# google/telluride_decoding

Hardware: AMD Instinct MI355X
Metric: TRF-fit samples/sec (higher is better)
Workload: dtype f32 (every product as 3 float16 products of a 2-piece split on the f16 MFMA, f32 accumulate, f64 slab sums; f64 solve)

## Files before the change

telluride_decoding_amd/csrc/lagcov.hip:

```cpp
#include <cstdlib>
#include <cstring>

#include "td_common.h"

namespace {

typedef float f32x16 __attribute__((ext_vector_type(16)));

constexpr int kThreads = 256;
constexpr int kTile = 128;
constexpr int kTileG = 64;
constexpr int kNpfU = 10;
constexpr int kNpfU2 = 13;
constexpr int kNpfG = 9;
constexpr int kLagsPerWg = 8;
constexpr int kHalo = 8;
constexpr size_t kLagcovScratchCap = size_t(256) << 20;

__device__ __forceinline__ int xcd_remap(int bid, int nwg) {
  const int q = nwg >> 3, r = nwg & 7;
  const int xcd = bid & 7, within = bid >> 3;
  const int base = xcd < r ? xcd * (q + 1) : r * (q + 1) + (xcd - r) * q;
  return base + within;
}
// ... 140 lines not shown
    }
  };
  const int nfull = nk >> 1;
  float c[6], n[6];
  ld(0, c);
  int kk = 0;
  for (; kk + 1 < nfull; kk += 2) {
    ld(kk + 1, n);
    mm(c);
    ld(kk + 2 < nfull ? kk + 2 : kk + 1, c);
    mm(n);
  }
  if (kk < nfull) mm(c);
  if (nk & 1) {
    ld(nfull, c);
    if (lk) { c[0] = 0.f; c[1] = 0.f; }
    mm(c);
  }
}

template <int kTileT, bool kM2, bool kN2>
__device__ __forceinline__ void mfma_tile_few(const float* __restrict__ as,
                                              const float* __restrict__ bs, int wave, int lane,
                                              int nk, int g, int lg, f32x16 (&acc)[2][2][2]) {
  const int lr = lane & 31, lk = lane >> 5;
  const int s_phases = 8 >> lg;
  const int nfull = nk >> 1;
#pragma unroll
  for (int le = 0; le < 2; ++le) {
    const int slot = 2 * wave + le;
    const int lag = slot & (g - 1), phase = slot >> lg;
    const float* ap = as + lk * 64 + lr;
    const float* bp = bs + (lk + lag) * 64 + lr;
    auto step = [&](int kk, bool tail) {
      const bool live = !tail || lk == 0;
      const float a0 = live ? ap[kk * 128] : 0.f;
      const float a1 = (kM2 && live) ? ap[kk * 128 + 32] : 0.f;
      const float b0 = bp[kk * 128];
      acc[le][0][0] = __builtin_amdgcn_mfma_f32_32x32x2f32(a0, b0, acc[le][0][0], 0, 0, 0);
      if (kM2) acc[le][1][0] = __builtin_amdgcn_mfma_f32_32x32x2f32(a1, b0, acc[le][1][0], 0, 0, 0);
      if (kN2) {
        const float b1 = bp[kk * 128 + 32];
        acc[le][0][1] = __builtin_amdgcn_mfma_f32_32x32x2f32(a0, b1, acc[le][0][1], 0, 0, 0);
        if (kM2) acc[le][1][1] = __builtin_amdgcn_mfma_f32_32x32x2f32(a1, b1, acc[le][1][1], 0, 0, 0);
      }
    };
#pragma unroll 4
    for (int kk = phase; kk < nfull; kk += s_phases) step(kk, false);
    if ((nk & 1) && (nfull & (s_phases - 1)) == phase) step(nfull, true);
  }
}

template <bool kUnified, int kTileT, int kNPF, bool kVec4, bool kFew>
__global__ __launch_bounds__(kThreads, 2) void lagcov_mfma_kernel(LagParams p) {
  extern __shared__ __attribute__((aligned(16))) float lds[];

  const int tid = threadIdx.x;
  const int lane = tid & 63;
  const int wave = __builtin_amdgcn_readfirstlane(tid >> 6);

  int id = xcd_remap(blockIdx.x, gridDim.x);
  const int group = id % p.n_groups; id /= p.n_groups;
  const int cbt = id % p.n_cbt; id /= p.n_cbt;
  const int cat = id % p.n_cat; id /= p.n_cat;
  const LagWork w = p.works[id];
  const int e0 = p.e_min + group * (kFew ? p.lag_g : kLagsPerWg);

  const int rows = kUnified ? kTileT + kHalo + e0 : 2 * kTileT + kHalo;
  const float* as = lds;
  const float* bs = kUnified ? lds + e0 * 64 : lds + kTileT * 64;

  const int ca_eff = p.ca + p.a_ones;
  const bool m2 = ca_eff - cat * 64 > 32;
  const bool n2 = p.cb - cbt * 64 > 32;
  const int ones_col = p.a_ones ? p.ca - cat * 64 : -1;

  f32x16 acc[2][2][2];
#pragma unroll
  for (int i = 0; i < 2; ++i)
#pragma unroll
    for (int j = 0; j < 2; ++j)
#pragma unroll
      for (int k = 0; k < 2; ++k)
#pragma unroll
        for (int r = 0; r < 16; ++r) acc[i][j][k][r] = 0.f;

  float4 pf[kNPF];
  prefetch_tile<kUnified, kTileT, kNPF, kVec4>(p, w, w.u_begin, e0, rows, cat, cbt, tid, pf);
  store_tile<kUnified, kTileT, kNPF>(lds, w, w.u_begin, ones_col, tid, pf);
  __syncthreads();

  for (long long ut = w.u_begin; ut < w.u_end; ut += kTileT) {
    const bool more = ut + kTileT < w.u_end;
    if (more)
      prefetch_tile<kUnified, kTileT, kNPF, kVec4>(p, w, ut + kTileT, e0, rows, cat, cbt, tid,
                                                      pf);
    const long long left = w.u_end - ut;
    const int nk = (kUnified && left < kTileT) ? (int)left : kTileT;
    if (kFew) {
      if (m2) {
        if (n2) mfma_tile_few<kTileT, true, true>(as, bs, wave, lane, nk, p.lag_g, p.lag_lg, acc);
        else    mfma_tile_few<kTileT, true, false>(as, bs, wave, lane, nk, p.lag_g, p.lag_lg, acc);
      } else {
        if (n2) mfma_tile_few<kTileT, false, true>(as, bs, wave, lane, nk, p.lag_g, p.lag_lg, acc);
        else    mfma_tile_few<kTileT, false, false>(as, bs, wave, lane, nk, p.lag_g, p.lag_lg, acc);
      }
    } else if (m2) {
      if (n2) mfma_tile<kTileT, true, true>(as, bs, wave, lane, nk, acc);
      else    mfma_tile<kTileT, true, false>(as, bs, wave, lane, nk, acc);
    } else {
      if (n2) mfma_tile<kTileT, false, true>(as, bs, wave, lane, nk, acc);
      else    mfma_tile<kTileT, false, false>(as, bs, wave, lane, nk, acc);
    }
    if (more) {
      __syncthreads();
      store_tile<kUnified, kTileT, kNPF>(lds, w, ut + kTileT, ones_col, tid, pf);
      __syncthreads();
    }
  }

  const int lr = lane & 31, lk = lane >> 5;
  float* slab = p.partial + (size_t)id * p.e_pad * p.ca_pad * p.cb_pad;
#pragma unroll
  for (int le = 0; le < 2; ++le) {
    int e_idx = group * kLagsPerWg + 2 * wave + le;
    if (kFew) {
      const int slot = 2 * wave + le;
      e_idx = ((slot >> p.lag_lg) * p.n_groups + group) * p.lag_g + (slot & (p.lag_g - 1));
    }
    float* pe = slab + (size_t)e_idx * p.ca_pad * p.cb_pad;
#pragma unroll
    for (int m = 0; m < 2; ++m)
#pragma unroll
      for (int n = 0; n < 2; ++n)
#pragma unroll
        for (int r = 0; r < 16; ++r) {
          const int i = cat * 64 + m * 32 + (r & 3) + 8 * (r >> 2) + 4 * lk;
          const int j = cbt * 64 + n * 32 + lr;
          pe[(size_t)i * p.cb_pad + j] = acc[le][m][n][r];
        }
  }
}

constexpr int kBfTile = 128;
template <int kRowDw, int kPieces> struct BfGeom {
  static constexpr int kRows = kRowDw == 83 ? 160 : 192;
  static constexpr int kPieceDw = 64 * kRowDw;
  static constexpr size_t kLdsBytes =
      sizeof(unsigned) * (2 * kPieces * kPieceDw + (kPieces == 2 ? 2 * 2 * 96 + 8 * 1024 : 0));
};
constexpr int kBfThreads = 512;

typedef td_u32x4 u32x4;

__device__ __forceinline__ float comp4(const float4& v, int q) {
  return q == 0 ? v.x : q == 1 ? v.y : q == 2 ? v.z : v.w;
}

template <bool kZero, int kBfPieceDw, bool kF16>
__device__ __forceinline__ void bf_kstep(const unsigned* __restrict__ ap,
                                         const unsigned* __restrict__ bp,
                                         const unsigned* a_mask, f32x16 (&acc)[4]) {
  constexpr int kP = kF16 ? 2 : 3;
  u32x4 a[kP];
  unsigned d[kP][6];
#pragma unroll
  for (int pc = 0; pc < kP; ++pc) {
#pragma unroll
    for (int i = 0; i < 4; ++i) a[pc][i] = ap[pc * kBfPieceDw + i];
#pragma unroll
    for (int i = 0; i < 6; ++i) d[pc][i] = bp[pc * kBfPieceDw + i];
  }
  if (a_mask) {
#pragma unroll
    for (int pc = 0; pc < kP; ++pc)
#pragma unroll
      for (int i = 0; i < 4; ++i) a[pc][i] &= a_mask[i];
  }
  u32x4 b[4][kP];
#pragma unroll
  for (int pc = 0; pc < kP; ++pc)
#pragma unroll
    for (int i = 0; i < 4; ++i) {
      b[0][pc][i] = d[pc][i];
      b[1][pc][i] = __builtin_amdgcn_alignbit(d[pc][i + 1], d[pc][i], 16);
      b[2][pc][i] = d[pc][i + 1];
      b[3][pc][i] = __builtin_amdgcn_alignbit(d[pc][i + 2], d[pc][i + 1], 16);
    }
  f32x16 c[4];
#pragma unroll
  for (int r = 0; r < 4; ++r) {
    if (kZero) {
#pragma unroll
      for (int k = 0; k < 16; ++k) c[r][k] = 0.f;
    } else {
      c[r] = acc[r];
    }
  }
  if constexpr (kF16) {
    constexpr int pa[3] = {1, 0, 0}, pb[3] = {0, 1, 0};
#pragma unroll
    for (int t = 0; t < 3; ++t)
#pragma unroll
      for (int r = 0; r < 4; ++r) c[r] = td_mfma_f16(a[pa[t] % kP], b[r][pb[t] % kP], c[r]);
  } else {
    constexpr int pa[6] = {2, 0, 1, 1, 0, 0}, pb[6] = {0, 2, 1, 0, 1, 0};
#pragma unroll
    for (int t = 0; t < 6; ++t)
#pragma unroll
      for (int r = 0; r < 4; ++r) c[r] = td_mfma_bf16(a[pa[t] % kP], b[r][pb[t] % kP], c[r]);
  }
#pragma unroll
  for (int r = 0; r < 4; ++r) acc[r] = c[r];
}

template <int kFrom, int kTo, int kBfPieceDw, bool kF16, int kChain>
__device__ __forceinline__ void bf_ksteps(const unsigned* __restrict__ ap,
                                          const unsigned* __restrict__ bp, f32x16 (&acc)[4],
                                          f32x16 (&total)[4]) {
#pragma unroll
  for (int s = kFrom; s < kTo; ++s) {
    if (s % kChain == 0) bf_kstep<true, kBfPieceDw, kF16>(ap + 8 * s, bp + 8 * s, nullptr, acc);
    else                 bf_kstep<false, kBfPieceDw, kF16>(ap + 8 * s, bp + 8 * s, nullptr, acc);
    if ((s + 1) % kChain == 0) {
#pragma unroll
      for (int r = 0; r < 4; ++r) total[r] += acc[r];
    }
    __builtin_amdgcn_sched_barrier(0);
  }
}

template <bool kVec4, int kBfRowDw, bool kF16, bool kVirt = false, bool kKs = false>
__global__ __launch_bounds__(kBfThreads) void lagcov_split_kernel(LagParams p) {
  static_assert(!kVirt || kF16, "virtual images: the float16 form");
  static_assert(!kKs || kVirt, "shared tasks: virtual images");
  constexpr int kChain = 8;
  constexpr int kP = kF16 ? 2 : 3;
  extern __shared__ __attribute__((aligned(16))) unsigned ldsu[];
  constexpr int kBfRows = BfGeom<kBfRowDw, kP>::kRows;
  constexpr int kBfPieceDw = BfGeom<kBfRowDw, kP>::kPieceDw;

  const int tid = threadIdx.x;
  const int lane = tid & 63;
  const int wave = __builtin_amdgcn_readfirstlane(tid >> 6);
  int quad = wave & 1, mt = (wave >> 1) & 1, nt = wave >> 2;

  int id = xcd_remap(blockIdx.x, gridDim.x);
  const int group = id % p.n_groups; id /= p.n_groups;
  const int part = id;
  LagWork w = p.works[id];
  const int e0 = group * kLagsPerWg;
  int lag_off = e0 + 4 * quad, out_lag = lag_off;
  bool active = true, a_ext = false;
  const VirtImage* img = nullptr;
  VirtSeg vs = {0, 0, 0};
  int kparts = 1, kq = 0;
  if constexpr (kVirt) {
    const VirtGroup* vg = p.vgroups + group;
    const VirtTask tk = vg->task[wave];
    img = p.vimgs + vg->image;
    mt = tk.mt; nt = tk.nt; lag_off = tk.lag0; out_lag = tk.out_lag;
    active = out_lag >= 0; a_ext = tk.a_ext != 0;
    if constexpr (kKs) {
      kparts = __builtin_amdgcn_readfirstlane((int)tk.kparts);
      kq = __builtin_amdgcn_readfirstlane((int)tk.kq);
    }
    vs = p.vsegs[id];
  }
  const int ksn = 8 / kparts, ks0 = kq * ksn;

  f32x16 total[4];
#pragma unroll
  for (int r = 0; r < 4; ++r)
#pragma unroll
    for (int k = 0; k < 16; ++k) total[r][k] = 0.f;

  const int c4 = (tid & 15) * 4, rg = tid >> 4;
  const bool has_tail = kBfRows == 192 || wave < 4;
  const bool early = wave < 4;
  float sc[4] = {1.f, 1.f, 1.f, 1.f};
  int vdesc[4] = {0, 0, 0, 0};
  if constexpr (kVirt) {
#pragma unroll
    for (int q = 0; q < 4; ++q) {
      const int k = kVec4 ? c4 + q : lane;
      vdesc[q] = (img->src[k] + 1) | (img->role[k] ? 0x100 : 0) | ((int)img->shift[k] << 16);
    }
  }
  constexpr int kVPairs = kBfRows / 16;
  auto v_src = [&](int q) { return (vdesc[q] & 0xff) - 1; };
  auto v_sh = [&](int q) { return vdesc[q] >> 16; };
  auto v_role = [&](int q) { return (vdesc[q] & 0x100) != 0; };
  if (kF16) {
#pragma unroll
    for (int q = 0; q < 4; ++q) {
      const int ch = kVirt ? v_src(q) : min(c4 + q, 63);
      const int k = ch >= 0 ? td_f16_scale_exp(td_chan_max_of(p.chan_max, ch)) : 0;
      sc[q] = __builtin_bit_cast(float, (unsigned)(127 + k) << 23);
      if (kVirt && ch < 0) sc[q] = 0.f;
    }
    if (blockIdx.x == 0 && tid < 128) {
      unsigned* all = const_cast<unsigned*>(p.chan_max);
      const unsigned m = td_chan_max_of(p.chan_max, tid);
      all[kChanShards * 128 + tid] = m;
      if (p.scale_out) p.scale_out[tid] = m;
    }
    if (p.zero_tab && blockIdx.x == (gridDim.x > 1 ? 1 : 0))
      for (int i = tid; i < kChanTab; i += kBfThreads) p.zero_tab[i] = 0u;
  }
  const bool never = false;
  float anchor_a = 0.f, anchor_b = 1.f;
  auto sched_anchor = [&](unsigned* dst) {
    if (!never || tid >= 160) return;
    reinterpret_cast<unsigned short*>(dst)[tid] = (unsigned short)(anchor_a * anchor_b);
  };
  float4 pf[6];
  auto interior = [&](long long ut) -> bool {
    return kVec4 && p.ca == 64 && ut >= 0 && ut + kBfRows <= w.a_valid;
  };
  auto vrange = [&](long long ut, int q, int& lo, int& hi) {
    const long long lim = 1 << 20;
    const long long a0 = -ut, b0 = w.a_valid - ut;
    const long long a1 = vs.seg_begin - ut, b1 = (vs.seg_end < w.a_valid ? vs.seg_end : w.a_valid) - ut;
    const int a0i = (int)(a0 < -lim ? -lim : (a0 > lim ? lim : a0)), b0i = (int)(b0 < -lim ? -lim : (b0 > lim ? lim : b0));
    const int a1i = (int)(a1 < -lim ? -lim : (a1 > lim ? lim : a1)), b1i = (int)(b1 < -lim ? -lim : (b1 > lim ? lim : b1));
    lo = (v_role(q) ? a1i : a0i) - v_sh(q);
    hi = (v_role(q) ? b1i : b0i) - v_sh(q);
    if (v_src(q) < 0) { lo = 0; hi = 0; }
  };
  int v_min_shift = 0, v_max_shift = 0;
  bool v_any_role1 = false;
  if constexpr (kVirt) { v_min_shift = img->min_shift; v_max_shift = img->max_shift; v_any_role1 = img->any_role1 != 0; }
  auto vinside = [&](long long ut) -> bool {
    const long long lo = v_any_role1 && vs.seg_begin > 0 ? vs.seg_begin : 0;
    const long long hi = v_any_role1 && vs.seg_end < w.a_valid ? vs.seg_end : w.a_valid;
    return ut + v_min_shift >= lo && ut + kBfRows + v_max_shift <= hi;
  };
  auto prefetch_to = [&](long long ut, float4 (&pfr)[6]) {
    if constexpr (kVirt) {
      if (vinside(ut)) {
        const int ld = (int)p.lda;
        const float* base = p.a + (w.a_row0 + ut) * p.lda;
        if (kVec4) {
          const int off = (4 * rg + v_sh(0)) * ld + (v_src(0) < 0 ? 0 : v_src(0));
#pragma unroll
          for (int s = 0; s < 4; ++s) pfr[s] = *reinterpret_cast<const float4*>(base + s * ld + off);
          if (has_tail) {
            const float* tb = base + kBfTile * ld;
            const int toff = off - 2 * rg * ld;
#pragma unroll
            for (int s = 0; s < 2; ++s) pfr[4 + s] = *reinterpret_cast<const float4*>(tb + s * ld + toff);
          }
        } else {
          const int off = (2 * wave + v_sh(0)) * ld + (v_src(0) < 0 ? 0 : v_src(0));
          float* pv = reinterpret_cast<float*>(&pfr[0]);
#pragma unroll
          for (int j = 0; j < kVPairs; ++j) {
            pv[2 * j] = (base + 16 * j * ld)[off];
            pv[2 * j + 1] = (base + (16 * j + 1) * ld)[off];
          }
        }
        return;
      }
      const float* base = p.a + (w.a_row0 + ut) * p.lda;
      const int ld = (int)p.lda;
      const long long l0 = -ut, h0 = w.a_valid - 1 - ut, lim = 1 << 20;
      const int rlo = (int)(l0 < -lim ? -lim : (l0 > lim ? lim : l0));
      const int rhi = (int)(h0 < -lim ? -lim : (h0 > lim ? lim : h0));
      if (kVec4) {
        const int src = v_src(0) < 0 ? 0 : v_src(0), sh = v_sh(0);
#pragma unroll
        for (int s = 0; s < 4; ++s) {
          const int rc = max(rlo, min(4 * rg + s + sh, rhi));
          pfr[s] = *reinterpret_cast<const float4*>(base + rc * ld + src);
        }
        if (has_tail) {
#pragma unroll
          for (int s = 0; s < 2; ++s) {
            const int rc = max(rlo, min(kBfTile + 2 * rg + s + sh, rhi));
            pfr[4 + s] = *reinterpret_cast<const float4*>(base + rc * ld + src);
          }
        }
      } else {
        const int src = v_src(0) < 0 ? 0 : v_src(0), sh = v_sh(0);
        float* pv = reinterpret_cast<float*>(&pfr[0]);
#pragma unroll
        for (int j = 0; j < 2 * kVPairs; ++j) {
          const int r = 16 * (j >> 1) + 2 * wave + (j & 1);
          const int rc = max(rlo, min(r + sh, rhi));
          pv[j] = base[rc * ld + src];
        }
      }
      return;
    }
    if (interior(ut)) {
      const float* base = p.a + (w.a_row0 + ut) * p.lda + c4;
      const int ld = (int)p.lda;
#pragma unroll
      for (int s = 0; s < 4; ++s)
        pfr[s] = *reinterpret_cast<const float4*>(base + (4 * rg + s) * ld);
      if (has_tail) {
#pragma unroll
        for (int s = 0; s < 2; ++s)
          pfr[4 + s] = *reinterpret_cast<const float4*>(base + (kBfTile + 2 * rg + s) * ld);
      }
      return;
    }
    const RowWindow rw = row_window(p.a, p.lda, w.a_row0, ut, w.a_valid, 0, p.ca);
#pragma unroll
    for (int s = 0; s < 4; ++s) pfr[s] = load_row4_raw<kVec4>(rw, 4 * rg + s, c4);
    if (has_tail) {
#pragma unroll
      for (int s = 0; s < 2; ++s) pfr[4 + s] = load_row4_raw<kVec4>(rw, kBfTile + 2 * rg + s, c4);
    }
  };
  auto prefetch = [&](long long ut) { prefetch_to(ut, pf); };
  auto store_from = [&](long long ut, unsigned* buf, const float4 (&pfr)[6]) {
    if constexpr (kVirt && !kVec4) {
      const float* pv = reinterpret_cast<const float*>(&pfr[0]);
      unsigned* dst = buf + lane * kBfRowDw + wave;
      if (vinside(ut)) {
#pragma unroll
        for (int j = 0; j < kVPairs; ++j) {
          unsigned h, l;
          td_split2_f16(pv[2 * j] * sc[0], pv[2 * j + 1] * sc[0], h, l);
          dst[8 * j] = h;
          dst[kBfPieceDw + 8 * j] = l;
        }
        return;
      }
      int lo, hi;
      vrange(ut, 0, lo, hi);
#pragma unroll
      for (int j = 0; j < kVPairs; ++j) {
        const int r = 16 * j + 2 * wave;
        const float x0 = (r >= lo && r < hi) ? pv[2 * j] : 0.f;
        const float x1 = (r + 1 >= lo && r + 1 < hi) ? pv[2 * j + 1] : 0.f;
        unsigned h, l;
        td_split2_f16(x0 * sc[0], x1 * sc[0], h, l);
        dst[8 * j] = h;
        dst[kBfPieceDw + 8 * j] = l;
      }
      return;
    }
    float4 v[6];
#pragma unroll
    for (int s = 0; s < 6; ++s) v[s] = pfr[s];
    if constexpr (kVirt) {
      if (!vinside(ut))
#pragma unroll
      for (int q = 0; q < 4; ++q) {
        int lo, hi;
        vrange(ut, kVec4 ? 0 : q, lo, hi);
        if (lo <= 0 && hi >= kBfRows) continue;
#pragma unroll
        for (int s = 0; s < 4; ++s) {
          const int r = 4 * rg + s;
          float& x = reinterpret_cast<float*>(&v[s])[q];
          x = (r >= lo && r < hi) ? x : 0.f;
        }
#pragma unroll
        for (int s = 0; s < 2; ++s) {
          const int r = kBfTile + 2 * rg + s;
          float& x = reinterpret_cast<float*>(&v[4 + s])[q];
          x = (r >= lo && r < hi) ? x : 0.f;
        }
      }
    } else
    if (!interior(ut)) {
      const RowWindow rw = row_window(p.a, p.lda, w.a_row0, ut, w.a_valid, 0, p.ca);
#pragma unroll
      for (int s = 0; s < 4; ++s) v[s] = mask_row4(rw, 4 * rg + s, true, c4, pfr[s]);
      if (has_tail) {
#pragma unroll
        for (int s = 0; s < 2; ++s) v[4 + s] = mask_row4(rw, kBfTile + 2 * rg + s, true, c4, pfr[4 + s]);
      }
    }
#pragma unroll
    for (int q = 0; q < 4; ++q) {
      unsigned* dst = buf + (c4 + q) * kBfRowDw + 2 * rg;
      if (kF16) {
        unsigned h[2], l[2];
#pragma unroll
        for (int d = 0; d < 2; ++d)
          td_split2_f16(comp4(v[2 * d], q) * sc[q], comp4(v[2 * d + 1], q) * sc[q], h[d], l[d]);
        dst[0] = h[0]; dst[1] = h[1];
        dst[kBfPieceDw] = l[0]; dst[kBfPieceDw + 1] = l[1];
      } else {
        unsigned h[2], m[2], l[2];
#pragma unroll
        for (int d = 0; d < 2; ++d)
          td_split3(comp4(v[2 * d], q), comp4(v[2 * d + 1], q), h[d], m[d], l[d]);
        dst[0] = h[0]; dst[1] = h[1];
        dst[kBfPieceDw] = m[0]; dst[kBfPieceDw + 1] = m[1];
        dst[(kP - 1) * kBfPieceDw] = l[0]; dst[(kP - 1) * kBfPieceDw + 1] = l[1];
      }
    }
    if (has_tail) {
#pragma unroll
      for (int q = 0; q < 4; ++q) {
        unsigned* tail = buf + (c4 + q) * kBfRowDw + kBfTile / 2 + rg;
        if (kF16) {
          unsigned h, l;
          td_split2_f16(comp4(v[4], q) * sc[q], comp4(v[5], q) * sc[q], h, l);
          tail[0] = h;
          tail[kBfPieceDw] = l;
        } else {
          unsigned h, m, l;
          td_split3(comp4(v[4], q), comp4(v[5], q), h, m, l);
          tail[0] = h;
          tail[kBfPieceDw] = m;
          tail[(kP - 1) * kBfPieceDw] = l;
        }
      }
    }
  };
  auto store = [&](long long ut, unsigned* buf) { store_from(ut, buf, pf); };

  const int lj = lane & 31, lg = lane >> 5;
  const int a_off = (mt * 32 + lj) * kBfRowDw + 4 * lg;
  const int b_off = (nt * 32 + lj) * kBfRowDw + 4 * lg + (lag_off >> 1);

  f32x16 acc[4];
  unsigned* const buf0 = ldsu;
  unsigned* const buf1 = ldsu + kP * kBfPieceDw;
  for (; id < p.n_work; id += p.n_part) {
  if (id != part) {
    __syncthreads();
    w = p.works[id];
    if constexpr (kVirt) vs = p.vsegs[id];
  }
  if constexpr (kKs) {
    const long long u_stop = vs.u_end_ext;
    float4 pf2[6];
    prefetch_to(w.u_begin, pf);
    store_from(w.u_begin, buf0, pf);
    if (w.u_begin + kBfTile < u_stop) prefetch_to(w.u_begin + kBfTile, pf);
    __syncthreads();
    auto ks_tile = [&](long long ut, const unsigned* cur, unsigned* nxt, float4 (&pfa)[6], float4 (&pfb)[6]) {
      const bool more = ut + kBfTile < u_stop;
      if (ut + 2 * kBfTile < u_stop) prefetch_to(ut + 2 * kBfTile, pfb);
      long long left = (a_ext ? u_stop : w.u_end) - ut;
      if (!active) left = 0;
      const unsigned* ap = cur + a_off;
      const unsigned* bp = cur + b_off;
      if (left >= kBfTile) {
        bf_kstep<true, kBfPieceDw, kF16>(ap + 8 * ks0, bp + 8 * ks0, nullptr, acc);
        for (int s = ks0 + 1; s < ks0 + ksn; ++s)
          bf_kstep<false, kBfPieceDw, kF16>(ap + 8 * s, bp + 8 * s, nullptr, acc);
#pragma unroll
        for (int r = 0; r < 4; ++r) total[r] += acc[r];
      } else if (left > 16 * ks0) {
        const int nk = (int)left;
#pragma unroll
        for (int r = 0; r < 4; ++r)
#pragma unroll
          for (int k = 0; k < 16; ++k) acc[r][k] = 0.f;
        const int t_hi = min(nk, 16 * (ks0 + ksn));
        for (int t0 = 16 * ks0; t0 < t_hi; t0 += 16) {
          const int cnt = nk - t0 - 8 * lg;
          unsigned mask[4];
#pragma unroll
          for (int d = 0; d < 4; ++d)
            mask[d] = cnt >= 2 * d + 2 ? 0xffffffffu : cnt == 2 * d + 1 ? 0x0000ffffu : 0u;
          bf_kstep<false, kBfPieceDw, kF16>(ap + (t0 >> 1), bp + (t0 >> 1), mask, acc);
        }
#pragma unroll
        for (int r = 0; r < 4; ++r) total[r] += acc[r];
      }
      if (more) {
        store_from(ut + kBfTile, nxt, pfa);
        __syncthreads();
      }
    };
    for (long long ut = w.u_begin; ut < u_stop; ut += 2 * kBfTile) {
      ks_tile(ut, buf0, buf1, pf, pf2);
      if (ut + kBfTile < u_stop) ks_tile(ut + kBfTile, buf1, buf0, pf2, pf);
    }
    continue;
  }
  prefetch(w.u_begin);
  store(w.u_begin, buf0);
  __syncthreads();

  const long long u_stop = kVirt ? vs.u_end_ext : w.u_end;
  int parity = 0;
  for (long long ut = w.u_begin; ut < u_stop; ut += kBfTile, parity ^= 1) {
    const unsigned* cur = parity ? buf1 : buf0;
    unsigned* nxt = parity ? buf0 : buf1;
    const bool more = ut + kBfTile < u_stop;
    if (more) prefetch(ut + kBfTile);
    long long left = w.u_end - ut;
    if constexpr (kVirt) {
      if (a_ext) left = u_stop - ut;
      if (!active) left = 0;
      if (left < kBfTile && more) store(ut + kBfTile, nxt);
    }
    const unsigned* ap = cur + a_off;
    const unsigned* bp = cur + b_off;
    if (left >= kBfTile) {
      bf_ksteps<0, 2, kBfPieceDw, kF16, kChain>(ap, bp, acc, total);
      if (more && early) { store(ut + kBfTile, nxt); sched_anchor(nxt); }
      bf_ksteps<2, 6, kBfPieceDw, kF16, kChain>(ap, bp, acc, total);
      if (more && !early) { store(ut + kBfTile, nxt); sched_anchor(nxt); }
      bf_ksteps<6, 8, kBfPieceDw, kF16, kChain>(ap, bp, acc, total);
    } else {
      const int nk = (int)left;
#pragma unroll
      for (int r = 0; r < 4; ++r)
#pragma unroll
        for (int k = 0; k < 16; ++k) acc[r][k] = 0.f;
      for (int t0 = 0; t0 < nk; t0 += 16) {
        const int cnt = nk - t0 - 8 * lg;
        unsigned mask[4];
#pragma unroll
        for (int d = 0; d < 4; ++d)
          mask[d] = cnt >= 2 * d + 2 ? 0xffffffffu : cnt == 2 * d + 1 ? 0x0000ffffu : 0u;
        bf_kstep<false, kBfPieceDw, kF16>(ap + (t0 >> 1), bp + (t0 >> 1), mask, acc);
      }
#pragma unroll
      for (int r = 0; r < 4; ++r) total[r] += acc[r];
    }
    if (more) __syncthreads();
  }
  }

  if constexpr (kKs) {
    float* const red = reinterpret_cast<float*>(ldsu);
    const int task = wave / kparts;
    for (int step = kparts >> 1; step >= 1; step >>= 1) {
      __syncthreads();
      if (kq >= step && kq < 2 * step) {
        float* dst = red + (size_t)(task * step + kq - step) * 4096 + lane;
#pragma unroll
        for (int r = 0; r < 4; ++r)
#pragma unroll
          for (int k = 0; k < 16; ++k) dst[(r * 16 + k) * 64] = total[r][k];
      }
      __syncthreads();
      if (kq < step) {
        const float* src = red + (size_t)(task * step + kq) * 4096 + lane;
#pragma unroll
        for (int r = 0; r < 4; ++r)
#pragma unroll
          for (int k = 0; k < 16; ++k) total[r][k] += src[(r * 16 + k) * 64];
      }
    }
    active = active && kq == 0;
  }
  if constexpr (kVirt) {
    if (active) {
      float* slab = p.partial + (size_t)part * p.slab_elems;
      const int lr = lane & 31, lk = lane >> 5;
#pragma unroll
      for (int r = 0; r < 4; ++r) {
        float* pe = slab + (size_t)(out_lag + r) * 1024;
#pragma unroll
        for (int k = 0; k < 16; ++k) pe[((k & 3) + 8 * (k >> 2) + 4 * lk) * 32 + lr] = total[r][k];
      }
    }
    return;
  }
  float* slab = p.partial + (size_t)part * p.e_pad * p.ca_pad * p.cb_pad;
#pragma unroll
  for (int r = 0; r < 4; ++r) {
    float* pe = slab + (size_t)(e0 + 4 * quad + r) * p.ca_pad * p.cb_pad;
    const int lr = lane & 31, lk = lane >> 5;
#pragma unroll
    for (int k = 0; k < 16; ++k) {
      const int i = mt * 32 + (k & 3) + 8 * (k >> 2) + 4 * lk;
      const int j = nt * 32 + lr;
      pe[(size_t)i * p.cb_pad + j] = total[r][k];
    }
  }
}

struct Narrow16Params {
  const float* x;
  const float* y;
  long long ldx, ldy;
  int c, d, pre, l1;
  const LagWork* works;
  int n_lg, lpw;
  int do_main, do_tgt;
  float* part;
  float* tpart;
  double* csum;
  double* ysum;
  long long n_part;
};

typedef float n16_f32x4 __attribute__((ext_vector_type(4)));

__device__ __forceinline__ float n16_load(__amdgpu_buffer_rsrc_t rs, unsigned voff) {
  return __builtin_bit_cast(float, __builtin_amdgcn_raw_buffer_load_b32(rs, (int)voff, 0, 0));
}

template <bool kMain, bool kTgt, int kLpw, int kD, bool kPre>
__global__ __launch_bounds__(256) void lagcov_narrow16_kernel(Narrow16Params p) {
  const int tid = threadIdx.x, lane = tid & 63;
  const int wave = __builtin_amdgcn_readfirstlane(tid >> 6);
  const int g = wave % p.n_lg, sub = wave / p.n_lg, n_sub = 4 / p.n_lg;
  const LagWork w = p.works[blockIdx.x];
  const long long len = w.u_end - w.u_begin;
  const long long sub_len = ((len + n_sub - 1) / n_sub + 3) / 4 * 4;
  const long long ub = w.u_begin + sub * sub_len;
  const long long ue = ub + sub_len < w.u_end ? ub + sub_len : w.u_end;
  const int j = lane & 15, k = lane >> 4;
  const int e0 = g * kLpw;
  const int ne = p.l1 - e0 < kLpw ? p.l1 - e0 : kLpw;
  const __amdgpu_buffer_rsrc_t rx = __builtin_amdgcn_make_buffer_rsrc(
      const_cast<float*>(p.x + w.b_row0 * p.ldx), 0,
      w.b_valid > 0 ? (int)(((w.b_valid - 1) * p.ldx + p.c) * 4) : 0, 0x00020000);
  const __amdgpu_buffer_rsrc_t ry = __builtin_amdgcn_make_buffer_rsrc(
      const_cast<float*>(p.y + w.a_row0 * p.ldy), 0,
      w.a_valid > 0 ? (int)(((w.a_valid - 1) * p.ldy + p.d) * 4) : 0, 0x00020000);
  const unsigned row_x = (unsigned)(p.ldx * 4), row_y = (unsigned)(p.ldy * 4);
  const unsigned lane_x = j < p.c ? (unsigned)k * row_x + 4u * j : 0x80000000u;
  const unsigned lane_y = (unsigned)k * row_y;
  const unsigned lag0 = (unsigned)e0 * row_x, pre_x = (unsigned)p.pre * row_x;
  n16_f32x4 acc[kLpw];
  float tacc[kD][kLpw];
#pragma unroll
  for (int q = 0; q < kLpw; ++q) {
    acc[q] = n16_f32x4{0.f, 0.f, 0.f, 0.f};
#pragma unroll
    for (int col = 0; col < kD; ++col) tacc[col][q] = 0.f;
  }
  float cs = 0.f, ys[kD];
#pragma unroll
  for (int col = 0; col < kD; ++col) ys[col] = 0.f;
  constexpr int kU = kLpw >= 8 ? 2 : 4;
  for (long long u = ub; u < ue; u += 4 * kU) {
    const unsigned vx = lane_x + (unsigned)u * row_x;
    const unsigned vy = lane_y + (unsigned)u * row_y;
    float a[kU], b[kU][kLpw], bt[kU][kLpw], yv[kU][kD];
#pragma unroll
    for (int st = 0; st < kU; ++st) {
      const unsigned vs = vx + (unsigned)(4 * st) * row_x;
      a[st] = n16_load(rx, vs);
#pragma unroll
      for (int q = 0; q < kLpw; ++q) b[st][q] = n16_load(rx, vs + lag0 + (unsigned)q * row_x);
      if (kTgt) {
#pragma unroll
        for (int col = 0; col < kD; ++col) yv[st][col] = n16_load(ry, vy + (unsigned)(4 * st) * row_y + 4u * col);
        if (kPre) {
#pragma unroll
          for (int q = 0; q < kLpw; ++q) bt[st][q] = n16_load(rx, vs + lag0 + (unsigned)q * row_x - pre_x);
        }
      }
    }
#pragma unroll
    for (int st = 0; st < kU; ++st) {
      const bool in_slab = k + 4 * st < ue - u;
      const float av = in_slab ? a[st] : 0.f;
#pragma unroll
      for (int q = 0; q < kLpw; ++q) {
        if (kMain) acc[q] = __builtin_amdgcn_mfma_f32_16x16x4f32(av, b[st][q], acc[q], 0, 0, 0);
        if (kTgt) {
#pragma unroll
          for (int col = 0; col < kD; ++col) {
            const float yc = in_slab ? yv[st][col] : 0.f;
            tacc[col][q] += yc * (kPre ? bt[st][q] : b[st][q]);
          }
        }
      }
      if (kTgt) {
        cs += av;
#pragma unroll
        for (int col = 0; col < kD; ++col) ys[col] += in_slab ? yv[st][col] : 0.f;
      }
    }
  }
  constexpr int kSlot = kLpw * 256 + kD * kLpw * 16 + 16 + 16;
  __shared__ float red[3 * kSlot];
  if (kTgt) {
#pragma unroll
    for (int col = 0; col < kD; ++col) {
#pragma unroll
      for (int q = 0; q < kLpw; ++q) {
        float t = tacc[col][q];
        t += __shfl_xor(t, 16);
        t += __shfl_xor(t, 32);
        tacc[col][q] = t;
      }
      float t = ys[col];
      t += __shfl_xor(t, 16);
      t += __shfl_xor(t, 32);
      ys[col] = t;
    }
    cs += __shfl_xor(cs, 16);
    cs += __shfl_xor(cs, 32);
  }
  if (sub > 0) {
    float* slot = red + ((sub - 1) * p.n_lg + g) * kSlot;
    if (kMain) {
#pragma unroll
      for (int q = 0; q < kLpw; ++q)
#pragma unroll
        for (int r = 0; r < 4; ++r) slot[(q * 4 + r) * 64 + lane] = acc[q][r];
    }
    if (kTgt && k == 0) {
#pragma unroll
      for (int col = 0; col < kD; ++col) {
#pragma unroll
        for (int q = 0; q < kLpw; ++q) slot[kLpw * 256 + (col * kLpw + q) * 16 + j] = tacc[col][q];
        if (j == 0) slot[kLpw * 256 + kD * kLpw * 16 + 16 + col] = ys[col];
      }
      slot[kLpw * 256 + kD * kLpw * 16 + j] = cs;
    }
  }
  __syncthreads();
  if (sub > 0) return;
  for (int o = 1; o < n_sub; ++o) {
    const float* slot = red + ((o - 1) * p.n_lg + g) * kSlot;
    if (kMain) {
#pragma unroll
      for (int q = 0; q < kLpw; ++q)
#pragma unroll
// ... 2627 lines not shown
```

telluride_decoding_amd/csrc/td_common.h:

```cpp
#pragma once

#include <hip/hip_runtime.h>

#include <cstdarg>
#include <cstdint>
#include <cstdio>
#include <cstring>
#include <string>
#include <vector>

#include "td_hotpath.h"


constexpr int kChanShards = 16;
constexpr int kChanTab = (kChanShards + 1) * 128;

struct td_handle {
  int device = 0;
  int acc_mode = 0;
  int cu_count = 0;
  bool lds_opt_lagcov = false, lds_opt_virt = false, lds_opt_fir = false, lds_opt_fir_stream = false, lds_opt_proj_stream = false;
  hipStream_t own_stream = nullptr;
  hipStream_t stream = nullptr;
  hipEvent_t ev_start = nullptr, ev_stop = nullptr;
  hipEvent_t order_event = nullptr;
  std::string error;
  void* scratch = nullptr;
  size_t scratch_bytes = 0;
  void* work = nullptr;
  size_t work_bytes = 0;
  struct PinSlot {
    void* p = nullptr;
    size_t bytes = 0;
    hipEvent_t ev = nullptr;
    bool used = false;
  };
  static constexpr int kPinSlots = 16;
  PinSlot pin[kPinSlots];
  int pin_next = 0;
  struct TableSlot {
    void* dev = nullptr;
    size_t cap = 0;
    std::vector<char> host;
    uint64_t stamp = 0;
  };
  static constexpr int kTableSlots = 8;
  TableSlot tables[kTableSlots];
  uint64_t table_clock = 0;
  int* dev_flag = nullptr;
  unsigned* chan_max = nullptr;
  int chan_phase = 0;
  static constexpr int kAsyncFlags = 8;
  int* dev_flags = nullptr;
  int* host_flags = nullptr;
  int async_next = 0;
  hipEvent_t async_events[kAsyncFlags] = {};
  unsigned long long* cg_packets = nullptr;
  unsigned long long* cgt_packets = nullptr;
  unsigned cg_epoch = 0, cgt_epoch = 0;
  int* cg_status = nullptr;
  int solver_mode = 0;
  int cca_whitening = 0;
  int cca_fused = 1;
  bool lds_opt_cca = false, lds_opt_lu = false;
  long long cg_limit_ticks = -1;
  int async_cg = 0;
  int narrow16 = 1;
  int targets_f16 = 1;
  int last_solver = 0, last_iterations = 0, last_cg_status = 0;
  bool profile = false;
  std::vector<hipEvent_t> prof_events;
  size_t prof_used = 0;
  double prof_samples = 0;
};

int td_profile_mark(td_handle* h, bool start, double samples);

extern thread_local std::string td_global_error;

int td_fail(td_handle* h, int code, const char* fmt, ...);

#define TD_HIP(h, expr)                                                         \
  do {                                                                          \
    hipError_t _e = (expr);                                                     \
    if (_e != hipSuccess)                                                       \
      return td_fail((h), TD_ERR_HIP, "%s failed: %s (%s:%d)", #expr,           \
                     hipGetErrorString(_e), __FILE__, __LINE__);                \
  } while (0)

#define TD_TRY(expr)            \
  do {                          \
    int _s = (expr);            \
    if (_s != TD_OK) return _s; \
  } while (0)

#define TD_REQUIRE(h, cond, ...) \
  do {                           \
    if (!(cond)) return td_fail((h), TD_ERR_INVALID, __VA_ARGS__); \
  } while (0)

int td_scratch(td_handle* h, size_t bytes, void** out);

struct StatsCompact {
  bool ok;
  const double *fxx, *gxo, *sy;
  const float* win;
  int c, l, d, hw;
  int64_t n_files, frames;
};
int td_stats_compact(const td_stats* s, StatsCompact* out);
int td_cg_solve_compact(td_handle* h, const StatsCompact& sc, const double* lams_dev, const double* lams_host,
                        int n_lambda, int max_iter, double tol, double accept, float* w_dev, float* b_dev,
                        int* status_dev, int* flag_dev);
int td_cg_rows(int k, int cus);
constexpr int TD_CG_NOT_RESIDENT = 1;
int td_cg_solve_dense(td_handle* h, const double* xtx, int n, int ld, const double* xty, int d, double inv,
                      const double* lams_dev, int n_lambda, int cus, int max_iter, double tol, float* w_dev,
                      float* b_dev, int* status_dev, double accept = 100.0, bool gate = false);

int td_workspace(td_handle* h, size_t bytes, void** out);
int td_alloc_async(td_handle* h, size_t bytes, void** out);
int td_free_async(td_handle* h, void* p, bool own_stream_only = false);
int td_order_after_others(td_handle* h);

int td_upload_async(td_handle* h, const void* host, size_t bytes, void* dev_dst);

int td_table_upload(td_handle* h, const void* host, size_t bytes, const void** dev);

typedef __bf16 td_bf16x8 __attribute__((ext_vector_type(8)));
typedef __bf16 td_bf16x2 __attribute__((ext_vector_type(2)));
typedef float td_f32x2 __attribute__((ext_vector_type(2)));
typedef float td_f32x16 __attribute__((ext_vector_type(16)));
typedef unsigned td_u32x4 __attribute__((ext_vector_type(4)));

__device__ __forceinline__ unsigned td_pack_bf16(float a, float b) {
  const td_f32x2 v = {a, b};
  return __builtin_bit_cast(unsigned, __builtin_convertvector(v, td_bf16x2));
}

__device__ __forceinline__ void td_split3(float x0, float x1, unsigned& h, unsigned& m, unsigned& l) {
  h = td_pack_bf16(x0, x1);
  const float r0 = x0 - __builtin_bit_cast(float, h << 16);
  const float r1 = x1 - __builtin_bit_cast(float, h & 0xffff0000u);
  m = td_pack_bf16(r0, r1);
  const float s0 = r0 - __builtin_bit_cast(float, m << 16);
  const float s1 = r1 - __builtin_bit_cast(float, m & 0xffff0000u);
  l = td_pack_bf16(s0, s1);
}

__device__ __forceinline__ td_f32x16 td_mfma_bf16(const td_u32x4& a, const td_u32x4& b,
                                                  const td_f32x16& c) {
  return __builtin_amdgcn_mfma_f32_32x32x16_bf16(__builtin_bit_cast(td_bf16x8, a),
                                                 __builtin_bit_cast(td_bf16x8, b), c, 0, 0, 0);
}

typedef _Float16 td_f16x8 __attribute__((ext_vector_type(8)));
typedef _Float16 td_f16x2 __attribute__((ext_vector_type(2)));

__device__ __forceinline__ unsigned td_pack_f16(float a, float b) {
  const td_f32x2 v = {a, b};
  return __builtin_bit_cast(unsigned, __builtin_convertvector(v, td_f16x2));
}

__device__ __forceinline__ void td_split2_f16(float x0, float x1, unsigned& h, unsigned& l) {
  x0 = __builtin_amdgcn_fmed3f(x0, -65504.f, 65504.f);
  x1 = __builtin_amdgcn_fmed3f(x1, -65504.f, 65504.f);
  h = td_pack_f16(x0, x1);
  const td_f16x2 hv = __builtin_bit_cast(td_f16x2, h);
  l = td_pack_f16(x0 - (float)hv[0], x1 - (float)hv[1]);
}

__device__ __forceinline__ td_f32x16 td_mfma_f16(const td_u32x4& a, const td_u32x4& b,
                                                 const td_f32x16& c) {
  return __builtin_amdgcn_mfma_f32_32x32x16_f16(__builtin_bit_cast(td_f16x8, a),
                                                __builtin_bit_cast(td_f16x8, b), c, 0, 0, 0);
}

__device__ __forceinline__ unsigned td_chan_max_of(const unsigned* tab, int ch) {
  unsigned m = 0u;
#pragma unroll
  for (int sh = 0; sh < kChanShards; ++sh) m = max(m, tab[sh * 128 + ch]);
  return m;
}

__host__ __device__ __forceinline__ bool td_chan_not_finite(unsigned max_bits) {
  return ((max_bits >> 23) & 0xff) == 0xff;
}

__host__ __device__ __forceinline__ int td_f16_scale_exp(unsigned max_bits) {
  const int e = (int)((max_bits >> 23) & 0xff);
  if (max_bits == 0 || e == 0xff) return 0;
  int k = 14 - (e - 127);
  return k > 126 ? 126 : (k < -126 ? -126 : k);
}

static inline int64_t td_ceil_div(int64_t a, int64_t b) { return (a + b - 1) / b; }
static inline int64_t td_round_up(int64_t a, int64_t b) { return td_ceil_div(a, b) * b; }

struct LagSeg {
  int64_t a_row0;
  int64_t a_valid;
  int64_t b_row0;
  int64_t b_valid;
  int64_t u_begin;
  int64_t u_end;
};

struct LagWork {
  long long a_row0, a_valid, b_row0, b_valid, u_begin, u_end;
};

struct LagParams {
  const float* a;
  const float* b;
  long long lda, ldb;
  int ca, cb;
  int a_ones;
  const LagWork* works;
  int n_work, n_groups, n_cat, n_cbt;
  int e_min, e_count;
  float* partial;
  int n_part;
  int e_pad, ca_pad, cb_pad;
  int lag_g, lag_lg;
  const unsigned* chan_max;
  unsigned* scale_out = nullptr;
  unsigned* zero_tab = nullptr;
  const struct VirtImage* vimgs = nullptr;
  const struct VirtGroup* vgroups = nullptr;
  const struct VirtSeg* vsegs = nullptr;
  long long slab_elems = 0;
};

struct VirtImage {
  short src[64];
  short shift[64];
  signed char role[64];
  short min_shift, max_shift;
  short any_role1, pad;
};
struct VirtTask {
  signed char mt, nt;
  signed char a_ext;
  signed char kparts;
  short lag0;
  short kq;
  int out_lag;
};
struct VirtGroup {
  int image;
  int pad;
  VirtTask task[8];
};
struct VirtSeg {
  long long seg_begin, seg_end;
  long long u_end_ext;
};
struct VirtPair {
  int slot0, E, da, db;
  short nsa, nsb, wa, wb, col_a, col_b;
};
struct VirtMap {
  VirtPair pair[4][4];
};
__host__ __device__ __forceinline__ long long td_virt_offset(const VirtMap* vm, int e, int i, int j, int* e1_out = nullptr) {
  const VirtPair& P = vm->pair[i >> 5][j >> 5];
  int sb = e / P.db;
  sb = sb < P.nsb - 1 ? sb : P.nsb - 1;
  const int rem = e - sb * P.db;
  int sa = rem / P.da;
  sa = sa < P.nsa - 1 ? sa : P.nsa - 1;
  const int e1 = rem - sa * P.da;
  if (e1_out) *e1_out = e1;
  return ((long long)(P.slot0 + e1) * 32 + P.col_a + sa * P.wa + (i & 31)) * 32 + P.col_b + sb * P.wb + (j & 31);
}

struct LagReduceJob {
  const void* partial;
  int is_f64;
  int n_work, e_pad, ca_pad, cb_pad, e_count, ca_eff, cb;
  double* g;
  int accumulate, ca_dst, ldg;
  int mirror;
  const unsigned* scale_a;
  const unsigned* scale_b;
  const struct VirtMap* vmap = nullptr;
// ... 129 lines not shown
```

Before: 1.177 billion.

## Hand-schedule split-product MFMA k-steps in inline asm with a 7-lag B span

Adds an inline-assembly k-step for the lag-covariance split kernel. Each wave loads a 7-dword B window per piece and forms the odd-lag operands with v_alignbit shifts in registers instead of separate loads, then interleaves the shifts with the f16/bf16 MFMAs. In the non-virtual path a quad's lags now start two apart instead of four, remapped through bf_lag_of, and per-piece base pointers are precomputed. The accumulator hazard drain (s_nop) runs only at the end of each chain. The cost is hard-coded register allocation with clobbered VGPRs and hand-placed hazard nops, which raises register pressure and makes correctness depend on exact MFMA latencies.

Measured after the change: 1.183 billion (median of 6 runs). About the same (+0.5%).

```diff
diff --git a/telluride_decoding_amd/csrc/lagcov.hip b/telluride_decoding_amd/csrc/lagcov.hip
--- a/telluride_decoding_amd/csrc/lagcov.hip
+++ b/telluride_decoding_amd/csrc/lagcov.hip
@@ -316,12 +316,126 @@
 constexpr int kBfThreads = 512;
 
 typedef td_u32x4 u32x4;
+typedef td_u32x6 u32x6;
 
 __device__ __forceinline__ float comp4(const float4& v, int q) {
   return q == 0 ? v.x : q == 1 ? v.y : q == 2 ? v.z : v.w;
 }
 
-template <bool kZero, int kBfPieceDw, bool kF16>
+#define TD_CIN_ACC(n) "%" #n
+#define TD_CIN_ZERO(n) "0"
+#define TD_MF(op, n, a, b, cin) op " %" #n ", " a ", " b ", " cin "\n"
+#define TD_SH(p, hi, lo) "v_alignbit_b32 v" #p ", " hi ", v" #lo ", 16\n"
+#define TD_LAG_F16 "v_mfma_f32_32x32x16_f16"
+#define TD_LAG_BF16 "v_mfma_f32_32x32x16_bf16"
+#define TD_LAG_KSTEP_F16(CIN)                                                                      \
+  "s_nop 1\n"                                                                                      \
+  TD_MF(TD_LAG_F16, 0, "%5", "v[0:3]", CIN(0))                                                     \
+  TD_SH(8, "v1", 0) TD_SH(9, "v2", 1) TD_SH(10, "v3", 2) TD_SH(11, "v4", 3)                        \
+  TD_MF(TD_LAG_F16, 2, "%5", "v[2:5]", CIN(2))                                                     \
+  TD_SH(12, "v5", 4) TD_SH(13, "%6", 5) TD_SH(24, "v17", 16) TD_SH(25, "v18", 17)                  \
+  TD_MF(TD_LAG_F16, 1, "%5", "v[8:11]", CIN(1))                                                    \
+  TD_SH(26, "v19", 18) TD_SH(27, "v20", 19)                                                        \
+  TD_MF(TD_LAG_F16, 3, "%5", "v[10:13]", CIN(3))                                                   \
+  TD_SH(28, "v21", 20) TD_SH(29, "%7", 21)                                                         \
+  TD_MF(TD_LAG_F16, 0, "%4", "v[16:19]", "%0") TD_MF(TD_LAG_F16, 2, "%4", "v[18:21]", "%2")        \
+  TD_MF(TD_LAG_F16, 1, "%4", "v[24:27]", "%1") TD_MF(TD_LAG_F16, 3, "%4", "v[26:29]", "%3")        \
+  TD_MF(TD_LAG_F16, 0, "%4", "v[0:3]", "%0") TD_MF(TD_LAG_F16, 1, "%4", "v[8:11]", "%1")           \
+  TD_MF(TD_LAG_F16, 2, "%4", "v[2:5]", "%2") TD_MF(TD_LAG_F16, 3, "%4", "v[10:13]", "%3")
+#define TD_LAG_BF16_PC0(a)                                                                         \
+  TD_MF(TD_LAG_BF16, 0, a, "v[0:3]", "%0") TD_MF(TD_LAG_BF16, 1, a, "v[8:11]", "%1")               \
+  TD_MF(TD_LAG_BF16, 2, a, "v[2:5]", "%2") TD_MF(TD_LAG_BF16, 3, a, "v[10:13]", "%3")
+#define TD_LAG_BF16_PC1(a)                                                                         \
+  TD_MF(TD_LAG_BF16, 0, a, "v[16:19]", "%0") TD_MF(TD_LAG_BF16, 2, a, "v[18:21]", "%2")            \
+  TD_MF(TD_LAG_BF16, 1, a, "v[24:27]", "%1") TD_MF(TD_LAG_BF16, 3, a, "v[26:29]", "%3")
+#define TD_LAG_KSTEP_BF16(CIN)                                                                     \
+  "s_nop 1\n"                                                                                      \
+  TD_MF(TD_LAG_BF16, 0, "%6", "v[0:3]", CIN(0))                                                    \
+  TD_SH(8, "v1", 0) TD_SH(9, "v2", 1) TD_SH(10, "v3", 2) TD_SH(11, "v4", 3)                        \
+  TD_MF(TD_LAG_BF16, 2, "%6", "v[2:5]", CIN(2))                                                    \
+  TD_SH(12, "v5", 4) TD_SH(13, "%7", 5) TD_SH(40, "v33", 32) TD_SH(41, "v34", 33)                  \
+  TD_MF(TD_LAG_BF16, 1, "%6", "v[8:11]", CIN(1))                                                   \
+  TD_SH(42, "v35", 34) TD_SH(43, "v36", 35)                                                        \
+  TD_MF(TD_LAG_BF16, 3, "%6", "v[10:13]", CIN(3))                                                  \
+  TD_SH(44, "v37", 36) TD_SH(45, "%9", 37)                                                         \
+  TD_MF(TD_LAG_BF16, 0, "%4", "v[32:35]", "%0")                                                    \
+  TD_SH(24, "v17", 16) TD_SH(25, "v18", 17)                                                        \
+  TD_MF(TD_LAG_BF16, 2, "%4", "v[34:37]", "%2")                                                    \
+  TD_SH(26, "v19", 18) TD_SH(27, "v20", 19)                                                        \
+  TD_MF(TD_LAG_BF16, 1, "%4", "v[40:43]", "%1")                                                    \
+  TD_SH(28, "v21", 20) TD_SH(29, "%8", 21)                                                         \
+  TD_MF(TD_LAG_BF16, 3, "%4", "v[42:45]", "%3")                                                    \
+  TD_LAG_BF16_PC1("%5") TD_LAG_BF16_PC0("%5") TD_LAG_BF16_PC1("%4") TD_LAG_BF16_PC0("%4")
+#define TD_LAG_TMP_PC0 "v8", "v9", "v10", "v11", "v12", "v13"
+#define TD_LAG_TMP_PC1 "v24", "v25", "v26", "v27", "v28", "v29"
+#define TD_LAG_TMP_PC2 "v40", "v41", "v42", "v43", "v44", "v45"
+
+__device__ __forceinline__ constexpr int bf_lag_of(int r) { return (r & 1) + 4 * (r >> 1); }
+
+template <int kP> struct BfPieces {
+  const unsigned* p[kP];
+  __device__ __forceinline__ BfPieces operator+(int k) const {
+    BfPieces r;
+#pragma unroll
+    for (int pc = 0; pc < kP; ++pc) r.p[pc] = p[pc] + k;
+    return r;
+  }
+};
+
+__device__ __forceinline__ void bf_kstep_drain(f32x16 (&acc)[4]) {
+  asm volatile("s_nop 15\ns_nop 3" : "+v"(acc[0]), "+v"(acc[1]), "+v"(acc[2]), "+v"(acc[3]));
+}
+
+template <bool kZero, int kBfPieceDw, bool kF16, bool kDrain = true>
+__device__ __forceinline__ void bf_kstep(const BfPieces<kF16 ? 2 : 3>& ap, const BfPieces<kF16 ? 2 : 3>& bp,
+                                         const unsigned* a_mask, f32x16 (&acc)[4]) {
+  constexpr int kP = kF16 ? 2 : 3;
+  u32x4 a[kP];
+  u32x6 d[kP];
+  unsigned d6[kP];
+#pragma unroll
+  for (int pc = 0; pc < kP; ++pc) {
+#pragma unroll
+    for (int i = 0; i < 4; ++i) a[pc][i] = ap.p[pc][i];
+#pragma unroll
+    for (int i = 0; i < 6; ++i) d[pc][i] = bp.p[pc][i];
+    d6[pc] = bp.p[pc][6];
+  }
+  if (a_mask) {
+#pragma unroll
+    for (int pc = 0; pc < kP; ++pc)
+#pragma unroll
+      for (int i = 0; i < 4; ++i) a[pc][i] &= a_mask[i];
+  }
+  if constexpr (kF16) {
+    if constexpr (kZero)
+      asm volatile(TD_LAG_KSTEP_F16(TD_CIN_ZERO)
+                   : "=&v"(acc[0]), "=&v"(acc[1]), "=&v"(acc[2]), "=&v"(acc[3])
+                   : "v"(a[0]), "v"(a[1]), "v"(d6[0]), "v"(d6[1]), "{v[0:5]}"(d[0]), "{v[16:21]}"(d[1])
+                   : TD_LAG_TMP_PC0, TD_LAG_TMP_PC1);
+    else
+      asm volatile(TD_LAG_KSTEP_F16(TD_CIN_ACC)
+                   : "+v"(acc[0]), "+v"(acc[1]), "+v"(acc[2]), "+v"(acc[3])
+                   : "v"(a[0]), "v"(a[1]), "v"(d6[0]), "v"(d6[1]), "{v[0:5]}"(d[0]), "{v[16:21]}"(d[1])
+                   : TD_LAG_TMP_PC0, TD_LAG_TMP_PC1);
+  } else {
+    if constexpr (kZero)
+      asm volatile(TD_LAG_KSTEP_BF16(TD_CIN_ZERO)
+                   : "=&v"(acc[0]), "=&v"(acc[1]), "=&v"(acc[2]), "=&v"(acc[3])
+                   : "v"(a[0]), "v"(a[1]), "v"(a[kP - 1]), "v"(d6[0]), "v"(d6[1]), "v"(d6[kP - 1]),
+                     "{v[0:5]}"(d[0]), "{v[16:21]}"(d[1]), "{v[32:37]}"(d[kP - 1])
+                   : TD_LAG_TMP_PC0, TD_LAG_TMP_PC1, TD_LAG_TMP_PC2);
+    else
+      asm volatile(TD_LAG_KSTEP_BF16(TD_CIN_ACC)
+                   : "+v"(acc[0]), "+v"(acc[1]), "+v"(acc[2]), "+v"(acc[3])
+                   : "v"(a[0]), "v"(a[1]), "v"(a[kP - 1]), "v"(d6[0]), "v"(d6[1]), "v"(d6[kP - 1]),
+                     "{v[0:5]}"(d[0]), "{v[16:21]}"(d[1]), "{v[32:37]}"(d[kP - 1])
+                   : TD_LAG_TMP_PC0, TD_LAG_TMP_PC1, TD_LAG_TMP_PC2);
+  }
+  if constexpr (kDrain) bf_kstep_drain(acc);
+}
+
+template <bool kZero, int kBfPieceDw, bool kF16, bool kDrain = true>
 __device__ __forceinline__ void bf_kstep(const unsigned* __restrict__ ap,
                                          const unsigned* __restrict__ bp,
                                          const unsigned* a_mask, f32x16 (&acc)[4]) {
@@ -378,14 +492,14 @@
   for (int r = 0; r < 4; ++r) acc[r] = c[r];
 }
 
-template <int kFrom, int kTo, int kBfPieceDw, bool kF16, int kChain>
-__device__ __forceinline__ void bf_ksteps(const unsigned* __restrict__ ap,
-                                          const unsigned* __restrict__ bp, f32x16 (&acc)[4],
+template <int kFrom, int kTo, int kBfPieceDw, bool kF16, int kChain, class Op>
+__device__ __forceinline__ void bf_ksteps(const Op& ap, const Op& bp, f32x16 (&acc)[4],
                                           f32x16 (&total)[4]) {
 #pragma unroll
   for (int s = kFrom; s < kTo; ++s) {
-    if (s % kChain == 0) bf_kstep<true, kBfPieceDw, kF16>(ap + 8 * s, bp + 8 * s, nullptr, acc);
-    else                 bf_kstep<false, kBfPieceDw, kF16>(ap + 8 * s, bp + 8 * s, nullptr, acc);
+    if (s % kChain == 0)            bf_kstep<true, kBfPieceDw, kF16, false>(ap + 8 * s, bp + 8 * s, nullptr, acc);
+    else if ((s + 1) % kChain != 0) bf_kstep<false, kBfPieceDw, kF16, false>(ap + 8 * s, bp + 8 * s, nullptr, acc);
+    else                            bf_kstep<false, kBfPieceDw, kF16, true>(ap + 8 * s, bp + 8 * s, nullptr, acc);
     if ((s + 1) % kChain == 0) {
 #pragma unroll
       for (int r = 0; r < 4; ++r) total[r] += acc[r];
@@ -399,7 +513,9 @@
   static_assert(!kVirt || kF16, "virtual images: the float16 form");
   static_assert(!kKs || kVirt, "shared tasks: virtual images");
   constexpr int kChain = 8;
+  static_assert(kChain > 1, "bf_ksteps: a chain's first step is not its last");
   constexpr int kP = kF16 ? 2 : 3;
+  constexpr bool kSpan7 = !kVirt;
   extern __shared__ __attribute__((aligned(16))) unsigned ldsu[];
   constexpr int kBfRows = BfGeom<kBfRowDw, kP>::kRows;
   constexpr int kBfPieceDw = BfGeom<kBfRowDw, kP>::kPieceDw;
@@ -414,7 +530,7 @@
   const int part = id;
   LagWork w = p.works[id];
   const int e0 = group * kLagsPerWg;
-  int lag_off = e0 + 4 * quad, out_lag = lag_off;
+  int lag_off = e0 + (kSpan7 ? 2 : 4) * quad, out_lag = lag_off;
   bool active = true, a_ext = false;
   const VirtImage* img = nullptr;
   VirtSeg vs = {0, 0, 0};
@@ -684,6 +800,35 @@
   const int lj = lane & 31, lg = lane >> 5;
   const int a_off = (mt * 32 + lj) * kBfRowDw + 4 * lg;
   const int b_off = (nt * 32 + lj) * kBfRowDw + 4 * lg + (lag_off >> 1);
+  int a_offs[kP], b_offs[kP];
+  if constexpr (kSpan7) {
+#pragma unroll
+    for (int pc = 0; pc < kP; ++pc) {
+      a_offs[pc] = a_off + pc * kBfPieceDw;
+      b_offs[pc] = b_off + pc * kBfPieceDw;
+      if constexpr (kF16) asm volatile("" : "+v"(a_offs[pc]), "+v"(b_offs[pc]));
+    }
+  }
+  auto a_stream = [&](const unsigned* cur) {
+    if constexpr (kSpan7) {
+      BfPieces<kP> s;
+#pragma unroll
+      for (int pc = 0; pc < kP; ++pc) s.p[pc] = cur + a_offs[pc];
+      return s;
+    } else {
+      return cur + a_off;
+    }
+  };
+  auto b_stream = [&](const unsigned* cur) {
+    if constexpr (kSpan7) {
+      BfPieces<kP> s;
+#pragma unroll
+      for (int pc = 0; pc < kP; ++pc) s.p[pc] = cur + b_offs[pc];
+      return s;
+    } else {
+      return cur + b_off;
+    }
+  };
 
   f32x16 acc[4];
   unsigned* const buf0 = ldsu;
@@ -706,8 +851,8 @@
       if (ut + 2 * kBfTile < u_stop) prefetch_to(ut + 2 * kBfTile, pfb);
       long long left = (a_ext ? u_stop : w.u_end) - ut;
       if (!active) left = 0;
-      const unsigned* ap = cur + a_off;
-      const unsigned* bp = cur + b_off;
+      const auto ap = a_stream(cur);
+      const auto bp = b_stream(cur);
       if (left >= kBfTile) {
         bf_kstep<true, kBfPieceDw, kF16>(ap + 8 * ks0, bp + 8 * ks0, nullptr, acc);
         for (int s = ks0 + 1; s < ks0 + ksn; ++s)
@@ -760,8 +905,8 @@
       if (!active) left = 0;
       if (left < kBfTile && more) store(ut + kBfTile, nxt);
     }
-    const unsigned* ap = cur + a_off;
-    const unsigned* bp = cur + b_off;
+    const auto ap = a_stream(cur);
+    const auto bp = b_stream(cur);
     if (left >= kBfTile) {
       bf_ksteps<0, 2, kBfPieceDw, kF16, kChain>(ap, bp, acc, total);
       if (more && early) { store(ut + kBfTile, nxt); sched_anchor(nxt); }
@@ -828,7 +973,7 @@
   float* slab = p.partial + (size_t)part * p.e_pad * p.ca_pad * p.cb_pad;
 #pragma unroll
   for (int r = 0; r < 4; ++r) {
-    float* pe = slab + (size_t)(e0 + 4 * quad + r) * p.ca_pad * p.cb_pad;
+    float* pe = slab + (size_t)(lag_off + bf_lag_of(r)) * p.ca_pad * p.cb_pad;
     const int lr = lane & 31, lk = lane >> 5;
 #pragma unroll
     for (int k = 0; k < 16; ++k) {
diff --git a/telluride_decoding_amd/csrc/td_common.h b/telluride_decoding_amd/csrc/td_common.h
--- a/telluride_decoding_amd/csrc/td_common.h
+++ b/telluride_decoding_amd/csrc/td_common.h
@@ -132,6 +132,7 @@
 typedef float td_f32x2 __attribute__((ext_vector_type(2)));
 typedef float td_f32x16 __attribute__((ext_vector_type(16)));
 typedef unsigned td_u32x4 __attribute__((ext_vector_type(4)));
+typedef unsigned td_u32x6 __attribute__((ext_vector_type(6)));
 
 __device__ __forceinline__ unsigned td_pack_bf16(float a, float b) {
   const td_f32x2 v = {a, b};
```
